# LepistaBioinformatics/blutils

Measured on AMD Instinct MI355X. Metric: Mqueries/sec consensus (synthetic outfmt-6 hit table), higher is better.
Workload: dtype i32/u32

## Files before the change

### blutils_amd/csrc/consensus_kernel.hip

```cpp

#if defined(__HIP_DEVICE_COMPILE__) && !defined(__gfx950__)
#error "consensus_kernel.hip is written for gfx950"
#endif

#include <hip/hip_runtime.h>

#include <climits>
#include <cstdint>
#include <type_traits>

#include "blu_internal.h"

namespace blu {

#define WAVE 64

constexpr int BLOCK_A = 768;
constexpr int BLU_WAVES_PER_SIMD = 3;
constexpr int BLOCK_N = 1024;
constexpr int BLU_N_WAVES_PER_SIMD = 4;
constexpr int BLOCK_F = 704;
constexpr int LIST_CAP = 208;
constexpr int LIST_CAP_F64 = 232;
constexpr uint32_t SHORT_SEG = 128u;
constexpr uint32_t MAX_TASK_SEG = 512u;
constexpr uint32_t BLU_LONG_COST = 96u;
constexpr uint32_t BLU_DENSE_Q = 3u;
constexpr int BLU_STEP_SETS = 2;
constexpr uint32_t FLAT_ROWS = 8u;
constexpr uint32_t FLAT_SEG = 64u * FLAT_ROWS;
constexpr uint32_t FLAT_STEPS = 8u;
constexpr uint32_t FLAT_DEPTH = 4u;
constexpr uint32_t RING_ROWS = 2048u;
constexpr uint32_t RING_PAD = 32u;
constexpr uint32_t RING_CHUNKS = RING_ROWS / 256u;
constexpr uint32_t RING_MASK = RING_ROWS - 1u;
constexpr int STREAM_AUX = 0;
#define RING_DMA_MOD " sc1 nt"
constexpr int GATHER_AUX = 2;
constexpr int RECORD_AUX = 18;
constexpr int BLOCK_B = 256;
constexpr int BLU_B_WAVES_PER_SIMD = 7;

__device__ __forceinline__ int lane_id() { return (int)__builtin_amdgcn_mbcnt_hi(~0u, __builtin_amdgcn_mbcnt_lo(~0u, 0u)); }

template <int CTRL>
__device__ __forceinline__ int dpp(int v) { return __builtin_amdgcn_update_dpp(0, v, CTRL, 0xF, 0xF, true); }

#define ROW_REDUCE(x, OP)            \
    x = OP(x, dpp<0xB1>(x));         \
    x = OP(x, dpp<0x4E>(x));         \
    x = OP(x, dpp<0x124>(x));        \
    x = OP(x, dpp<0x128>(x));

__device__ __forceinline__ int imax(int a, int b) { return a > b ? a : b; }
__device__ __forceinline__ int imin(int a, int b) { return a < b ? a : b; }
__device__ __forceinline__ uint32_t umin(uint32_t a, uint32_t b) { return a < b ? a : b; }
__device__ __forceinline__ int rl(int v, int lane) { return __builtin_amdgcn_readlane(v, lane); }

__device__ __forceinline__ int wave_max_i32(int x) {
    ROW_REDUCE(x, imax)
    return imax(imax(rl(x, 0), rl(x, 16)), imax(rl(x, 32), rl(x, 48)));
}
__device__ __forceinline__ int wave_min_i32(int x) {
    ROW_REDUCE(x, imin)
    return imin(imin(rl(x, 0), rl(x, 16)), imin(rl(x, 32), rl(x, 48)));
}
__device__ __forceinline__ int iadd(int a, int b) { return a + b; }
__device__ __forceinline__ int wave_sum_u32(uint32_t v) {
    int x = (int)v;
    ROW_REDUCE(x, iadd)
    return rl(x, 0) + rl(x, 16) + rl(x, 32) + rl(x, 48);
}
__device__ __forceinline__ uint32_t wave_max_u32(uint32_t v) { return (uint32_t)wave_max_i32((int)(v ^ 0x80000000u)) ^ 0x80000000u; }
__device__ __forceinline__ uint32_t wave_min_u32(uint32_t v) { return (uint32_t)wave_min_i32((int)(v ^ 0x80000000u)) ^ 0x80000000u; }

__device__ __forceinline__ uint32_t wave_incl_scan_u32(uint32_t v) {
    uint32_t incl = v;
    incl += (uint32_t)dpp<0x111>((int)incl);
    incl += (uint32_t)dpp<0x112>((int)incl);
    incl += (uint32_t)dpp<0x114>((int)incl);
    incl += (uint32_t)dpp<0x118>((int)incl);
    const uint32_t t0 = (uint32_t)rl((int)incl, 15), t1 = (uint32_t)rl((int)incl, 31), t2 = (uint32_t)rl((int)incl, 47);
    const uint32_t r16 = (uint32_t)lane_id() >> 4;
    return incl + (r16 == 0 ? 0u : (r16 == 1 ? t0 : (r16 == 2 ? t0 + t1 : t0 + t1 + t2)));
}
#define WL_QUEUES 64u
#define WL_BASE 64u
#define WL_STRIDE 32u
__device__ __forceinline__ uint32_t wl_capacity(uint64_t n_queries) {
    const uint64_t n_tasks = (n_queries + WAVE - 1) / WAVE;
    return (uint32_t)((n_tasks + WL_QUEUES - 1) / WL_QUEUES) * WAVE;
}
__device__ __forceinline__ void wl_push(uint32_t* const wl_q, uint32_t* const wl_cnt, const uint32_t q) {
    __hip_atomic_store(wl_q + atomicAdd(wl_cnt, 1u), q, __ATOMIC_RELAXED, __HIP_MEMORY_SCOPE_AGENT);
}
__device__ __forceinline__ uint32_t wl_entry(const uint32_t* __restrict__ worklist, const uint32_t cap, const uint32_t incl, const uint32_t wi) {
    const uint32_t sub = (uint32_t)__builtin_popcountll(__ballot(incl <= wi));
    const uint32_t before = sub ? (uint32_t)rl((int)incl, (int)sub - 1) : 0u;
    return __hip_atomic_load(worklist + (uint64_t)sub * cap + (wi - before), __ATOMIC_RELAXED, __HIP_MEMORY_SCOPE_AGENT);
}

template <int CTRL>
__device__ __forceinline__ double dpp_f64(double v) {
    return __hiloint2double(dpp<CTRL>(__double2hiint(v)), dpp<CTRL>(__double2loint(v)));
}
__device__ __forceinline__ double rl_f64(double v, int lane) {
    return __hiloint2double(rl(__double2hiint(v), lane), rl(__double2loint(v), lane));
}
__device__ __forceinline__ double dmax(double a, double b) { return b > a ? b : a; }
__device__ __forceinline__ double dmin(double a, double b) { return b < a ? b : a; }
__device__ __forceinline__ double wave_max_f64(double x) {
    x = dmax(x, dpp_f64<0xB1>(x)); x = dmax(x, dpp_f64<0x4E>(x));
    x = dmax(x, dpp_f64<0x124>(x)); x = dmax(x, dpp_f64<0x128>(x));
    return dmax(dmax(rl_f64(x, 0), rl_f64(x, 16)), dmax(rl_f64(x, 32), rl_f64(x, 48)));
}
__device__ __forceinline__ double wave_min_f64(double x) {
    x = dmin(x, dpp_f64<0xB1>(x)); x = dmin(x, dpp_f64<0x4E>(x));
    x = dmin(x, dpp_f64<0x124>(x)); x = dmin(x, dpp_f64<0x128>(x));
    return dmin(dmin(rl_f64(x, 0), rl_f64(x, 16)), dmin(rl_f64(x, 32), rl_f64(x, 48)));
}
__device__ __forceinline__ int first_lane(uint64_t m) { return __builtin_ctzll(m); }
__device__ __forceinline__ int last_lane(uint64_t m) { return 63 - __builtin_clzll(m); }
__device__ __forceinline__ uint64_t rl_u64(uint64_t v, int lane) {
    return (uint64_t)(uint32_t)rl((int)(uint32_t)v, lane) | ((uint64_t)(uint32_t)rl((int)(uint32_t)(v >> 32), lane) << 32);
}
__device__ __forceinline__ uint64_t uniform64(uint64_t v) {
    return (uint64_t)(uint32_t)__builtin_amdgcn_readfirstlane((uint32_t)v) |
           ((uint64_t)(uint32_t)__builtin_amdgcn_readfirstlane((uint32_t)(v >> 32)) << 32);
}

__device__ __forceinline__ void store_result(blu_result* out, uint64_t q, uint32_t status, uint32_t flags,
                                             uint32_t bean_index, uint32_t mar_level, uint32_t reached_rank,
                                             uint32_t mar_code, uint32_t identifier, uint32_t ref_row,
                                             uint64_t level_mask, double ident) {
    uint4 a;
    a.x = (status & 0xFF) | ((flags & 0xFF) << 8) | ((bean_index & 0xFF) << 16) | ((mar_level & 0xFF) << 24);
    a.y = (reached_rank & 0xFFFF) | ((mar_code & 0xFFFF) << 16);
    a.z = identifier;
    a.w = ref_row;
    uint4 b;
    b.x = (uint32_t)level_mask;
    b.y = (uint32_t)(level_mask >> 32);
    b.z = (uint32_t)__double2loint(ident);
    b.w = (uint32_t)__double2hiint(ident);
    uint4* p = reinterpret_cast<uint4*>(out + q);
    p[0] = a;
    p[1] = b;
}
__device__ __forceinline__ void pack_result(uint4& a, uint4& b, uint32_t status, uint32_t flags, uint32_t bean_index,
                                            uint32_t mar_level, uint32_t reached_rank, uint32_t mar_code, uint32_t identifier,
                                            uint32_t ref_row, uint64_t level_mask, double ident) {
    a.x = (status & 0xFF) | ((flags & 0xFF) << 8) | ((bean_index & 0xFF) << 16) | ((mar_level & 0xFF) << 24);
    a.y = (reached_rank & 0xFFFF) | ((mar_code & 0xFFFF) << 16);
    a.z = identifier;
    a.w = ref_row;
    b.x = (uint32_t)level_mask;
    b.y = (uint32_t)(level_mask >> 32);
    b.z = (uint32_t)__double2loint(ident);
    b.w = (uint32_t)__double2hiint(ident);
}
__device__ __forceinline__ void pack_status(uint4& a, uint4& b, uint32_t status, uint32_t ref_row) {
    pack_result(a, b, status, 0, BLU_NONE_U8, BLU_NONE_U8, BLU_NONE_U16, BLU_NONE_U16, 0xFFFFFFFFu, ref_row, 0ull, 0.0);
}
__device__ __forceinline__ void store_status(blu_result* out, uint64_t q, uint32_t status, uint32_t ref_row) {
    store_result(out, q, status, 0, BLU_NONE_U8, BLU_NONE_U8, BLU_NONE_U16, BLU_NONE_U16, 0xFFFFFFFFu, ref_row, 0ull, 0.0);
}

__device__ __forceinline__ double milli_to_f64(uint32_t k) { return (double)k / 1000.0; }
__device__ __forceinline__ double milli17_to_f64(uint32_t k) {
    const double x = (double)k, y = 0.001;
    const double q = x * y;
    const double r = __builtin_fma(-q, 1000.0, x);
    return __builtin_fma(r, y, q);
}

__device__ __forceinline__ uint32_t packed_rank(uint32_t p) { return (p >> BLU_PACK_CUT_BITS) & BLU_PACK_CODE_MASK; }
__device__ __forceinline__ uint32_t packed_mar(uint32_t p) {
    const uint32_t m = p >> (BLU_PACK_CUT_BITS + BLU_PACK_CODE_BITS);
    return m == BLU_PACK_NEVER ? BLU_MAR_NEVER_EQUAL : m;
// ... 608 lines not shown
                    const uint32_t oq = g - L.qs[q];
                    left = g < total ? (int)sg.y - (int)(UR * oq) : 0;
                    if (left > 0) { voff = (sg.x + UR * oq) * 4u; um = q | (oq << 6) | (umin((uint32_t)left, UR) << 12); }
                }
                lo4 = __builtin_amdgcn_raw_buffer_load_b128(rs_bs, voff, 0, STREAM_AUX);
                hi4 = __builtin_amdgcn_raw_buffer_load_b128(rs_bs, left > 4 ? voff + 16u : 0xFFFFFFF0u, 0, STREAM_AUX);
            };
            u32x4 ba[DEPTH], bb[DEPTH];
            uint32_t um[MAXS];
            int lmx[MAXS];
#pragma unroll
            for (uint32_t st = 0; st < MAXS; ++st) { um[st] = 0u; lmx[st] = INT_MIN; }
#pragma unroll
            for (uint32_t st = 0; st < DEPTH; ++st) issue(st, ba[st], bb[st], um[st]);
#pragma unroll
            for (uint32_t st = 0; st < MAXS; ++st) {
                if (st >= ns) break;
                const u32x4 va = ba[st % DEPTH], vb = bb[st % DEPTH];
                const uint32_t left = (um[st] >> 12) & 15u;
                const uint32_t v[8] = {va.x, va.y, va.z, va.w, vb.x, vb.y, vb.z, vb.w};
                int bsv[UR], mx = INT_MIN;
#pragma unroll
                for (uint32_t r = 0; r < UR; ++r) { bsv[r] = left > r ? (int)v[r] : INT_MIN; mx = imax(mx, bsv[r]); }
                uint32_t lmask = 0;
#pragma unroll
                for (uint32_t r = 0; r < UR; ++r) lmask |= (uint32_t)(left > r && bsv[r] == mx) << r;
                um[st] |= lmask << 16;
                lmx[st] = mx;
                if (left) atomicMax(&L.qm[um[st] & 63u], mx);
                if (st + DEPTH < MAXS) issue(st + DEPTH, ba[st % DEPTH], bb[st % DEPTH], um[st + DEPTH]);
            }
            __builtin_amdgcn_fence(__ATOMIC_RELEASE, "workgroup");
            __builtin_amdgcn_wave_barrier();
            __builtin_amdgcn_fence(__ATOMIC_ACQUIRE, "workgroup");
            uint32_t running = fill, q_cut = q_lim;
#pragma unroll
            for (uint32_t st = 0; st < MAXS; ++st) {
                if (st >= ns) break;
                const uint32_t q = um[st] & 63u, oq = (um[st] >> 6) & 63u;
                const bool have = ((um[st] >> 12) & 15u) != 0u;
                const int M = L.qm[q];
                const uint32_t tmask = (have && lmx[st] == M) ? (um[st] >> 16) & 0xFFu : 0u;
                const uint32_t c = (uint32_t)__builtin_popcount(tmask);
                uint32_t in2 = c;
                in2 += (uint32_t)dpp<0x111>((int)in2);
                in2 += (uint32_t)dpp<0x112>((int)in2);
                in2 += (uint32_t)dpp<0x114>((int)in2);
                in2 += (uint32_t)dpp<0x118>((int)in2);
                const uint32_t k0 = (uint32_t)rl((int)in2, 15), k1 = (uint32_t)rl((int)in2, 31), k2 = (uint32_t)rl((int)in2, 47), k3 = (uint32_t)rl((int)in2, 63);
                in2 += r16 == 0 ? 0u : (r16 == 1 ? k0 : (r16 == 2 ? k0 + k1 : k0 + k1 + k2));
                const uint32_t idx0 = running + in2 - c;
                if (have && oq == 0u) L.meta[q] = META_SLOW | idx0;
                if (c) atomicAdd(&L.qk[q], c);
                const bool over = have && idx0 + c > CAP;
                const uint64_t over_m = __ballot(over);
                const bool room = !over && c != 0u && (over_m == 0ull || (uint32_t)lane < (uint32_t)__builtin_ctzll(over_m));
                if (room) L.rec[idx0] = make_uint4(__builtin_bitreverse32(tmask), L.seg[q].x + UR * oq, UR * oq, 0u);
                if (over_m) { q_cut = (uint32_t)rl((int)q, __builtin_ctzll(over_m)); break; }
                running += k0 + k1 + k2 + k3;
            }
            __builtin_amdgcn_fence(__ATOMIC_RELEASE, "workgroup");
            __builtin_amdgcn_wave_barrier();
            __builtin_amdgcn_fence(__ATOMIC_ACQUIRE, "workgroup");
            const uint32_t m = L.meta[lane];
            if (rows != 0u && (uint32_t)lane < q_cut) L.meta[lane] = (m & 0xFFFFu) | (L.qk[lane] << 16);
            fill = q_cut < q_lim ? (L.meta[q_cut] & 0xFFFFu) : running;
            if (q_cut < WAVE) stop_q = q_cut;
            }
        };
        auto ring_mark_landed = [&](const uint32_t upto) {
            const uint32_t m0 = (ring_landed + RING_CHUNKS - 1u) & ~(RING_CHUNKS - 1u);
            if (m0 < upto) {
                if ((uint32_t)lane < RING_PAD) L.ring[RING_ROWS + lane] = L.ring[lane];
                __builtin_amdgcn_fence(__ATOMIC_RELEASE, "workgroup");
                __builtin_amdgcn_wave_barrier();
                __builtin_amdgcn_fence(__ATOMIC_ACQUIRE, "workgroup");
            }
            ring_landed = upto;
        };
        auto ring_refill = [&]() {
            if (ring_head < ring_tail) { ring_head = ring_tail; if (ring_landed < ring_tail) ring_landed = ring_tail; }
            const uint32_t lim = ring_end < ring_tail + RING_CHUNKS ? ring_end : ring_tail + RING_CHUNKS;
            if (ring_head < lim) { ring_dma_run(rs_ring, ring_c0, ring_head, lim); ring_head = lim; }
        };
        auto phase1_scan = [&](const auto rpl_c, const auto full_c, const uint32_t LPQ) {
            constexpr uint32_t RPL = decltype(rpl_c)::value;
            constexpr bool FULL = decltype(full_c)::value;
            static_assert(RPL <= RING_PAD && RPL <= 32u, "rows per lane");
            const uint32_t QPS = WAVE / LPQ;
            const uint32_t grp = (uint32_t)lane / LPQ, sub = ((uint32_t)lane & (LPQ - 1u)) * RPL, row16 = (uint32_t)lane >> 4;
            {
                const uint32_t cs = (uint32_t)((vbase + (uint32_t)rl((int)seg_x, (int)first_q)) >> 8);
                if (cs < ring_tail) { wait_vmcnt(0u); ring_head = ring_landed = ring_tail = cs; }
            }
            for (uint32_t qb = first_q / QPS * QPS; qb < nq; qb += QPS) {
                const uint32_t r_lo = (uint32_t)rl((int)seg_x, (int)(qb < first_q ? first_q : qb));
                const uint32_t qn = qb + QPS;
                const uint32_t r_hi = qn < nq ? (uint32_t)rl((int)seg_x, (int)qn) : task_nrows;
                ring_tail = (uint32_t)((vbase + r_lo) >> 8);
                ring_refill();
                if (r_hi > r_lo) {
                    const uint32_t need = (uint32_t)((vbase + r_hi - 1u) >> 8);
                    if (need >= ring_landed) { wait_vmcnt(ring_head - 1u - need); ring_mark_landed(need + 1u); }
                }
                const uint32_t qi = qb + grp;
                const uint2 sg = L.seg[qi];
                const int left0 = (sg.y > short_seg ? 0 : (int)sg.y) - (int)sub;
                const uint32_t over = (FULL && left0 > 0 && left0 < (int)RPL) ? RPL - (uint32_t)left0 : 0u;
                const uint32_t sub_e = sub - over;
                const int left = FULL ? (left0 > 0 ? (int)RPL : 0) : left0;
                const uint32_t row0 = sg.x + sub_e;
                const uint32_t a = ((uint32_t)vbase + L.vx[qi] + sub_e) & RING_MASK;
                int b[RPL];
#pragma unroll
                for (uint32_t i = 0; i < RPL; ++i) b[i] = (int)L.ring[a + i];
                asm volatile("s_waitcnt lgkmcnt(0)" ::: "memory");
#pragma unroll
                for (uint32_t i = 0; i < RPL; ++i) asm volatile("" : "+v"(b[i]));
                if (r_hi > r_lo) { ring_tail = (uint32_t)((vbase + r_hi) >> 8); ring_refill(); }
                int M = INT_MIN;
                if constexpr (FULL) {
#pragma unroll
                    for (uint32_t i = 0; i < RPL; ++i) M = imax(M, b[i]);
                    M = left > 0 ? M : INT_MIN;
                } else {
#pragma unroll
                    for (uint32_t i = 0; i < RPL; ++i) { b[i] = (int)i < left ? b[i] : INT_MIN; M = imax(M, b[i]); }
                }
                if (LPQ >= 2) M = imax(M, dpp<0xB1>(M));
                if (LPQ >= 4) M = imax(M, dpp<0x4E>(M));
                if (LPQ >= 8) M = imax(M, dpp<0x141>(M));
                if (LPQ >= 16) M = imax(M, dpp<0x140>(M));
                uint32_t mask = tie_mask<RPL>(b, M);
                mask = left > 0 ? mask : 0u;
                if constexpr (FULL) mask &= 0xFFFFFFFFu >> (32u - RPL + over);
                const uint32_t c = (uint32_t)__builtin_popcount(mask);
                uint32_t incl = c;
                incl += (uint32_t)dpp<0x111>((int)incl);
                incl += (uint32_t)dpp<0x112>((int)incl);
                incl += (uint32_t)dpp<0x114>((int)incl);
                incl += (uint32_t)dpp<0x118>((int)incl);
                const uint32_t k0 = (uint32_t)rl((int)incl, 15), k1 = (uint32_t)rl((int)incl, 31);
                const uint32_t k2 = (uint32_t)rl((int)incl, 47), k3 = (uint32_t)rl((int)incl, 63);
                const bool fits = fill + k0 + k1 + k2 + k3 <= CAP;
                const uint32_t p1 = fill + k0, p2 = p1 + k1, p3 = p2 + k2;
                const uint32_t rbase = row16 == 0 ? fill : (row16 == 1 ? p1 : (row16 == 2 ? p2 : p3));
                uint32_t gk = c;
                if (LPQ >= 2) gk += (uint32_t)dpp<0xB1>((int)gk);
                if (LPQ >= 4) gk += (uint32_t)dpp<0x4E>((int)gk);
                if (LPQ >= 8) gk += (uint32_t)dpp<0x141>((int)gk);
                if (LPQ >= 16) gk += (uint32_t)dpp<0x140>((int)gk);
                if (PID32 && !fits) {
                    __builtin_amdgcn_s_setprio(2);
                    uint64_t BK = 0;
                    uint32_t bacc = 0, bpos = 0, brow = 0, kmin = 0xFFFFFFFFu, pmax = 0, dlo = 0xFFFFFFFFu, dhi = 0, err = 0xFFFFFFFFu;
                    auto reset = [&]() { BK = 0; bacc = 0; bpos = 0; brow = 0; kmin = 0xFFFFFFFFu; pmax = 0; dlo = 0xFFFFFFFFu; dhi = 0; err = 0xFFFFFFFFu; };
                    auto better = [&](const uint64_t K, const uint32_t acc, const uint32_t pos, const uint64_t K2, const uint32_t acc2, const uint32_t pos2) {
                        const bool gt = (K > K2) | ((K == K2) & (acc > acc2)), eq = (K == K2) & (acc == acc2);
                        return STRAT == BLU_RELAXED ? (gt | (eq & (pos > pos2))) : ((!gt & !eq) | (eq & (pos < pos2)));
                    };
                    auto take_record = [&](const u32x4 rec, const uint32_t gp, const bool on) {
                        const uint32_t len = umin(rec.x >> BLU_ROW_BITS, t.max_depth), pos = rec.x & ROW_MASK;
                        const bool unmatched = pos >= t.n_tax, bad = !unmatched && (rec.x >> BLU_ROW_BITS) == 0;
                        const uint32_t e = (gp << 8) | (bad ? (uint32_t)BLU_ST_ERR_BAD_LINEAGE : (uint32_t)BLU_ST_ERR_UNMATCHED_TAXID);
                        err = (on && (unmatched | bad)) ? umin(err, e) : err;
                        const uint32_t pm = rec.y & ((1u << KEY_PID_BITS) - 1u);
                        const uint32_t k1 = (len << KEY_PID_BITS) | pm;
                        const uint64_t K = ((uint64_t)k1 << 32) | (rec.z ^ 0x80000000u);
                        const bool take = on & ((kmin == 0xFFFFFFFFu) | better(K, rec.w, gp, BK, bacc, bpos));
                        BK = take ? K : BK; bacc = take ? rec.w : bacc; bpos = take ? gp : bpos; brow = take ? pos : brow;
                        kmin = on ? umin(kmin, k1) : kmin;
                        const uint32_t pmo = pm | ((!PACKED && rec.y >= (1u << KEY_PID_BITS)) ? 0x80000000u : 0u);
                        pmax = (on && pmo > pmax) ? pmo : pmax;
                        dlo = on ? umin(dlo, pos) : dlo;
                        dhi = (on && pos > dhi) ? pos : dhi;
                    };
                    auto load_record = [&](const uint32_t row, const bool on) {
                        u32x4 r;
                        if (PACKED) r = __builtin_amdgcn_raw_buffer_load_b128(rs_tax, on ? row * 16u : 0xFFFFFFC0u, 0, GATHER_AUX);
                        else {
                            const uint32_t o4 = on ? row * 4u : 0xFFFFFFF0u;
                            r.x = __builtin_amdgcn_raw_buffer_load_b32(rs_tax, o4, 0, GATHER_AUX);
                            r.y = __builtin_amdgcn_raw_buffer_load_b32(rs_pid, o4, 0, GATHER_AUX);
                            r.z = __builtin_amdgcn_raw_buffer_load_b32(rs_aln, o4, 0, GATHER_AUX);
                            r.w = __builtin_amdgcn_raw_buffer_load_b32(rs_acc, o4, 0, GATHER_AUX);
                        }
                        return r;
                    };
                    auto merge = [&](auto ctrl) {
                        constexpr int C = decltype(ctrl)::value;
                        const uint64_t K2 = ((uint64_t)(uint32_t)dpp<C>((int)(uint32_t)(BK >> 32)) << 32) | (uint32_t)dpp<C>((int)(uint32_t)BK);
                        const uint32_t acc2 = (uint32_t)dpp<C>((int)bacc), pos2 = (uint32_t)dpp<C>((int)bpos), row2 = (uint32_t)dpp<C>((int)brow);
                        const uint32_t kmin2 = (uint32_t)dpp<C>((int)kmin);
                        const bool take = (kmin2 != 0xFFFFFFFFu) & ((kmin == 0xFFFFFFFFu) | better(K2, acc2, pos2, BK, bacc, bpos));
                        BK = take ? K2 : BK; bacc = take ? acc2 : bacc; bpos = take ? pos2 : bpos; brow = take ? row2 : brow;
                        kmin = umin(kmin, kmin2);
                        const uint32_t pm2 = (uint32_t)dpp<C>((int)pmax); pmax = pm2 > pmax ? pm2 : pmax;
                        dlo = umin(dlo, (uint32_t)dpp<C>((int)dlo));
                        const uint32_t hi2 = (uint32_t)dpp<C>((int)dhi); dhi = hi2 > dhi ? hi2 : dhi;
                        err = umin(err, (uint32_t)dpp<C>((int)err));
                    };
                    auto deliver = [&](const int src, const bool mine) {
                        const uint32_t f_khi = (uint32_t)__builtin_amdgcn_ds_bpermute(src, (int)(uint32_t)(BK >> 32));
                        const uint32_t f_pos = (uint32_t)__builtin_amdgcn_ds_bpermute(src, (int)bpos), f_row = (uint32_t)__builtin_amdgcn_ds_bpermute(src, (int)brow);
                        const uint32_t f_kmin = (uint32_t)__builtin_amdgcn_ds_bpermute(src, (int)kmin), f_pmax = (uint32_t)__builtin_amdgcn_ds_bpermute(src, (int)pmax);
                        const uint32_t f_lo = (uint32_t)__builtin_amdgcn_ds_bpermute(src, (int)dlo), f_hi = (uint32_t)__builtin_amdgcn_ds_bpermute(src, (int)dhi);
                        const uint32_t f_err = (uint32_t)__builtin_amdgcn_ds_bpermute(src, (int)err);
                        const bool got = mine && f_kmin != 0xFFFFFFFFu;
                        const bool g_ovf = got && (f_pmax & 0x80000000u) != 0u, g_err = got && !g_ovf && f_err != 0xFFFFFFFFu, g_ok = got && !g_ovf && !g_err;
                        dn_flag = g_ovf ? 3u : (g_err ? 2u : (g_ok ? 1u : dn_flag));
                        dn_err = g_err ? (f_err & 0xFFu) : dn_err;
                        dn_pos = g_err ? (f_err >> 8) : dn_pos;
                        if constexpr (PID32) { r_pid = g_ok ? (f_khi & ((1u << KEY_PID_BITS) - 1u)) : r_pid; max_pid = g_ok ? f_pmax : max_pid; }
                        r_len = g_ok ? (f_khi >> KEY_PID_BITS) : r_len; r_row = g_ok ? f_row : r_row; r_pos = g_ok ? f_pos : r_pos;
                        minlen = g_ok ? (f_kmin >> KEY_PID_BITS) : minlen; g_lo = g_ok ? f_lo : g_lo; g_hi = g_ok ? f_hi : g_hi;
                    };
                    const uint32_t tq = (uint32_t)lane;
                    const bool mine = tq >= qb && tq < qn && tq < nq;
                    const uint32_t own0 = (mine ? tq - qb : 0u) * LPQ;
                    if (LPQ <= 4u && BLU_DENSE_Q * (k0 + k1 + k2 + k3) >= r_hi - r_lo) {
                        const uint32_t c4 = (uint32_t)lane & 3u;
#pragma nounroll
                        for (uint32_t g = 0; g < 4u; ++g) {
                            const int own = (int)((16u * g + ((uint32_t)lane >> 2)) * 4u);
                            const uint32_t o_row0 = (uint32_t)__builtin_amdgcn_ds_bpermute(own, (int)row0);
                            const uint32_t o_mask = (uint32_t)__builtin_amdgcn_ds_bpermute(own, (int)mask);
                            const uint32_t o_sub = (uint32_t)__builtin_amdgcn_ds_bpermute(own, (int)sub_e);
                            if (__ballot(o_mask != 0u) == 0ull) continue;
                            reset();
                            constexpr uint32_t NF = PACKED ? 4u : 2u;
#pragma unroll
                            for (uint32_t b0 = 0; b0 < RPL; b0 += 4u * NF) {
                                if (__ballot(((o_mask >> (RPL - 4u * NF - b0)) & ((1u << (4u * NF)) - 1u)) != 0u) == 0ull) continue;
                                u32x4 rq[NF];
#pragma unroll
                                for (uint32_t j = 0; j < NF; ++j) {
                                    const uint32_t i = b0 + 4u * j + c4;
                                    rq[j] = load_record(o_row0 + i, ((o_mask >> (RPL - 1u - i)) & 1u) != 0u);
                                }
#pragma unroll
                                for (uint32_t j = 0; j < NF; ++j) {
                                    const uint32_t i = b0 + 4u * j + c4;
                                    take_record(rq[j], o_sub + i, ((o_mask >> (RPL - 1u - i)) & 1u) != 0u);
                                }
                            }
                            merge(std::integral_constant<int, 0xB1>());
                            merge(std::integral_constant<int, 0x4E>());
                            if (LPQ >= 2) merge(std::integral_constant<int, 0x141>());
                            if (LPQ >= 4) merge(std::integral_constant<int, 0x140>());
                            deliver((int)(((own0 & 15u) * 4u) * 4u), mine && (own0 >> 4) == g);
                        }
                    } else {
                        uint32_t m = mask;
                        while (__ballot(m != 0u)) {
                            u32x4 rq[4];
                            uint32_t gp[4];
#pragma unroll
                            for (int j = 0; j < 4; ++j) {
                                const bool on = m != 0u;
                                const uint32_t hb = on ? 31u - (uint32_t)__builtin_clz(m) : 0u, i = RPL - 1u - hb;
                                m = on ? (m & ~(1u << hb)) : 0u;
                                gp[j] = on ? sub_e + i : 0xFFFFFFFFu;
                                rq[j] = load_record(row0 + i, on);
                            }
#pragma unroll
                            for (int j = 0; j < 4; ++j) take_record(rq[j], gp[j], gp[j] != 0xFFFFFFFFu);
                        }
                        if (LPQ >= 2) merge(std::integral_constant<int, 0xB1>());
                        if (LPQ >= 4) merge(std::integral_constant<int, 0x4E>());
                        if (LPQ >= 8) merge(std::integral_constant<int, 0x141>());
                        if (LPQ >= 16) merge(std::integral_constant<int, 0x140>());
                        deliver((int)(own0 * 4u), mine);
                    }
                    {
                        const uint32_t f_gk = (uint32_t)__builtin_amdgcn_ds_bpermute((int)(own0 * 4u), (int)gk);
                        dn_k = (mine && dn_flag == 1u) ? f_gk : dn_k;
                    }
                    if (sub == 0 && gk != 0u) L.meta[qi] = META_DENSE;
                    __builtin_amdgcn_s_setprio(0);
                    continue;
                }
                uint32_t idx = rbase + incl - c;
                if (!fits) {
                    const uint32_t lane_o = (uint32_t)__builtin_ctzll(__ballot(idx + c > CAP));
                    const uint32_t qo = qb + lane_o / LPQ;
                    const bool taken = qi < qo;
                    if (sub == 0) L.meta[qi] = taken ? (idx | (gk << 16)) : META_SLOW;
                    if (taken && c) { L.rec[idx].x = mask << (32u - RPL); L.rec[idx].y = DESC_WORD1(RPL, row0, sub_e); }
                    fill = (uint32_t)rl((int)idx, (int)((qo - qb) * LPQ));
                    stop_q = qo;
                    wait_vmcnt(0u);
                    ring_head = ring_landed = ring_tail = (uint32_t)((vbase + (uint32_t)rl((int)seg_x, (int)qo)) >> 8);
                    break;
                }
                if (sub == 0) L.meta[qi] = idx | (gk << 16);
                fill = p3 + k3;
                static_assert((RPL == 16u || RPL == 32u) && SHORT_SEG <= 128u, "descriptor word of a lane");
                if (c) { L.rec[idx].x = mask << (32u - RPL); L.rec[idx].y = DESC_WORD1(RPL, row0, sub_e); }
            }
        };
        auto gather_list = [&](auto&& between) {
            constexpr int NG = (CAP + WAVE - 1) / WAVE;
            u32x4 g[NG];
            uint32_t ghi[NG], gpos[NG], ghint[NG];
            uint32_t carry = 0;
#pragma unroll
            for (int u = 0; u < NG; ++u) {
                g[u] = u32x4{0u, 0u, 0u, 0u}; ghi[u] = 0u; gpos[u] = 0u; ghint[u] = 0u;
                if ((uint32_t)u * WAVE >= fill_ring) continue;
                const uint32_t idx = (uint32_t)u * WAVE + (uint32_t)lane;
                const bool valid = idx < fill_ring;
                const uint32_t d0 = L.rec[idx < CAP ? idx : 0u].x;
                int s = (valid && d0 != 0u) ? (int)idx : 0;
                s = imax(s, dpp<0x111>(s));
                s = imax(s, dpp<0x112>(s));
                s = imax(s, dpp<0x114>(s));
                s = imax(s, dpp<0x118>(s));
                s = imax(s, __builtin_amdgcn_update_dpp(0, s, 0x142, 0xA, 0xF, false));
                s = imax(s, __builtin_amdgcn_update_dpp(0, s, 0x143, 0xC, 0xF, false));
                s = imax(s, (int)carry);
                carry = (uint32_t)rl(s, 63);
                const uint4 dd = L.rec[s];
                const uint32_t d0w = dd.x, d = dd.y;
                uint32_t r = idx - (uint32_t)s, x = scan_rpl == 32u ? d0w : d0w >> 16, i = 0;
                if (scan_rpl == 32u) {
                    const uint32_t h = x >> 16, ch = (uint32_t)__builtin_popcount(h);
                    const bool low = r >= ch;
                    r -= low ? ch : 0u; x = low ? (x & 0xFFFFu) : h; i += low ? 16u : 0u;
                }
                {
                    const uint32_t h = x >> 8, ch = (uint32_t)__builtin_popcount(h);
                    const bool low = r >= ch;
                    r -= low ? ch : 0u; x = low ? (x & 0xFFu) : h; i += low ? 8u : 0u;
                }
                {
                    const uint32_t h = x >> 4, ch = (uint32_t)__builtin_popcount(h);
                    const bool low = r >= ch;
                    r -= low ? ch : 0u; x = low ? (x & 0xFu) : h; i += low ? 4u : 0u;
                }
                {
                    const uint32_t h = x >> 2, ch = (uint32_t)__builtin_popcount(h);
                    const bool low = r >= ch;
                    r -= low ? ch : 0u; x = low ? (x & 0x3u) : h; i += low ? 2u : 0u;
                }
                i += (r >= (x >> 1)) ? 1u : 0u;
                const uint32_t row = (RING ? (d >> DESC_SUB_BITS) : d) + i;
                gpos[u] = (RING ? (d & ((1u << DESC_SUB_BITS) - 1u)) : dd.z) + i;
                if (PACKED) g[u] = __builtin_amdgcn_raw_buffer_load_b128(rs_tax, valid ? row * 16u : 0xFFFFFFC0u, 0, GATHER_AUX);
                else if (WIDE) {
                    g[u] = __builtin_amdgcn_raw_buffer_load_b128(rs_tax, valid ? row * 24u : 0xFFFFFFC0u, 0, GATHER_AUX);
                    const u32x2 p = __builtin_amdgcn_raw_buffer_load_b64(rs_tax, valid ? row * 24u + 16u : 0xFFFFFFE0u, 0, GATHER_AUX);
                    ghint[u] = g[u].y;
                    g[u].y = p.x; ghi[u] = p.y;
                } else {
                    const uint32_t o4 = valid ? row * 4u : 0xFFFFFFF0u;
                    g[u].x = __builtin_amdgcn_raw_buffer_load_b32(rs_tax, o4, 0, GATHER_AUX);
                    if (PID32) g[u].y = __builtin_amdgcn_raw_buffer_load_b32(rs_pid, o4, 0, GATHER_AUX);
                    else {
                        const u32x2 p = __builtin_amdgcn_raw_buffer_load_b64(rs_pid, valid ? row * 8u : 0xFFFFFFE0u, 0, GATHER_AUX);
                        g[u].y = p.x; ghi[u] = p.y;
                    }
                    g[u].z = __builtin_amdgcn_raw_buffer_load_b32(rs_aln, o4, 0, GATHER_AUX);
                    g[u].w = __builtin_amdgcn_raw_buffer_load_b32(rs_acc, o4, 0, GATHER_AUX);
                }
            }
            between();
            bool ovf = false;
            uint32_t gk[NG];
#pragma unroll
            for (int u = 0; u < NG; ++u) {
                const bool valid = (uint32_t)u * WAVE + (uint32_t)lane < fill_ring;
                if constexpr (PID32) { gk[u] = g[u].y & PM_MASK; ovf |= !PACKED && valid && g[u].y >= (1u << KEY_PID_BITS); }
                else {
                    const double p = __hiloint2double((int)ghi[u], (int)g[u].y);
                    const bool in_range = p >= 0.0 && p < 131.0705;
                    const uint32_t k = in_range ? (uint32_t)(p * 1000.0 + 0.5) : 0u;
                    const double back = milli17_to_f64(k);
                    gk[u] = k;
                    ovf |= valid && !(in_range && __double2hiint(back) == (int)ghi[u] && __double2loint(back) == (int)g[u].y && k < BLU_KTHR_NEVER);
                }
            }
            keyed = __ballot(ovf) == 0ull && fill == fill_ring;
            bool any_bad = false;
#pragma unroll
            for (int u = 0; u < NG; ++u) {
                const uint32_t idx = (uint32_t)u * WAVE + (uint32_t)lane;
                if (idx < fill_ring) {
                    if (keyed) {
                        const uint32_t len = umin(g[u].x >> BLU_ROW_BITS, t.max_depth);
                        any_bad |= len == 0u || (g[u].x & ROW_MASK) >= t.n_tax;
                        const uint32_t hint = (PID32 ? g[u].y : ghint[u]) >> KEY_PID_BITS;
                        L.rec[idx] = make_uint4((g[u].x & ROW_MASK) | ((hint >> 8) << BLU_ROW_BITS),
                                                (len << KEYED_LEN_SHIFT) | (gk[u] << KEYED_PID_SHIFT) | (hint & 0xFFu), g[u].z ^ 0x80000000u, g[u].w);
                    } else L.rec[idx] = make_uint4(g[u].x, g[u].y, g[u].z, g[u].w);
                    L.pq[idx] = (uint16_t)gpos[u];
                    if (!PID32) L.p1[idx] = ghi[u];
                }
            }
            keyed_bad = __ballot(any_bad) != 0ull;
        };
        bool pend = (uint32_t)lane < nq;
        uint32_t pend_before = WAVE + 1;
        if (RING && contiguous) {
            ring_c0 = (uint32_t)(vbase >> 8);
            rs_ring = ring_desc(ring_c0);
            ring_end = task_nrows ? (uint32_t)((vbase + task_nrows - 1u) >> 8) + 1u : ring_c0;
            if (pref_q0 != q0_32) ring_head = ring_landed = ring_c0;
            ring_tail = ring_c0;
        }
        for (;;) {
        fill = 0;
        stop_q = WAVE;
        bool ring_round = false;
        bool list_round = false;
        keyed = false;
        {
            const uint32_t rows = L.seg[lane].y;
            const uint64_t live = __ballot(rows != 0u);
            first_q = live ? (uint32_t)__builtin_ctzll(live) : 0u;
// ... 868 lines not shown
```

Before: 11370.

## Software-pipeline dense-step record gathers and balance sparse gathers across lane pairs

The dense path of the overflow step now runs one continuous loop over all owner groups, using a three-deep ring of record requests so loads for the next blocks are in flight while the current block is reduced. The running best result is packed into fewer registers (position and row share one word, max pid and min length share another), which cuts the cross-lane DPP and bpermute traffic during merge and deliver. The sparse path pairs adjacent lanes so each gathers half of the pair's hits from both ends, and it issues a configurable number of loads per round. In exchange the code is more complex, register pressure from the ring buffer rises, and correctness depends on the new bit-packing assumptions, which are guarded by static asserts.

New measurement: 11260. About the same (-0.9%).

```diff
diff --git a/blutils_amd/csrc/consensus_kernel.hip b/blutils_amd/csrc/consensus_kernel.hip
--- a/blutils_amd/csrc/consensus_kernel.hip
+++ b/blutils_amd/csrc/consensus_kernel.hip
@@ -26,6 +26,10 @@
 constexpr uint32_t MAX_TASK_SEG = 512u;
 constexpr uint32_t BLU_LONG_COST = 96u;
 constexpr uint32_t BLU_DENSE_Q = 3u;
+#ifndef BLU_SPARSE_REQ_X
+#define BLU_SPARSE_REQ_X 6u
+#endif
+constexpr uint32_t BLU_SPARSE_REQ = BLU_SPARSE_REQ_X;
 constexpr int BLU_STEP_SETS = 2;
 constexpr uint32_t FLAT_ROWS = 8u;
 constexpr uint32_t FLAT_SEG = 64u * FLAT_ROWS;
@@ -940,9 +944,15 @@
                 if (LPQ >= 16) gk += (uint32_t)dpp<0x140>((int)gk);
                 if (PID32 && !fits) {
                     __builtin_amdgcn_s_setprio(2);
+                    constexpr uint32_t PL_LEN_SHIFT = KEY_PID_BITS + 1u, PL_PID_MASK = (1u << PL_LEN_SHIFT) - 1u;
+                    static_assert(BLU_ROW_BITS + 7u <= 32u && SHORT_SEG <= 128u && PL_LEN_SHIFT + 7u <= 32u, "packed words of a dense step's running result");
                     uint64_t BK = 0;
-                    uint32_t bacc = 0, bpos = 0, brow = 0, kmin = 0xFFFFFFFFu, pmax = 0, dlo = 0xFFFFFFFFu, dhi = 0, err = 0xFFFFFFFFu;
-                    auto reset = [&]() { BK = 0; bacc = 0; bpos = 0; brow = 0; kmin = 0xFFFFFFFFu; pmax = 0; dlo = 0xFFFFFFFFu; dhi = 0; err = 0xFFFFFFFFu; };
+                    uint32_t bacc = 0, bw = 0, pl = 0, dlo = 0xFFFFFFFFu, dhi = 0, err = 0xFFFFFFFFu;
+                    auto reset = [&]() { BK = 0; bacc = 0; bw = 0; pl = 0; dlo = 0xFFFFFFFFu; dhi = 0; err = 0xFFFFFFFFu; };
+                    auto pl_max = [&](const uint32_t a, const uint32_t b) {
+                        const uint32_t pa = a & PL_PID_MASK, pb = b & PL_PID_MASK, la = a >> PL_LEN_SHIFT, lb = b >> PL_LEN_SHIFT;
+                        return (pa > pb ? pa : pb) | ((la > lb ? la : lb) << PL_LEN_SHIFT);
+                    };
                     auto better = [&](const uint64_t K, const uint32_t acc, const uint32_t pos, const uint64_t K2, const uint32_t acc2, const uint32_t pos2) {
                         const bool gt = (K > K2) | ((K == K2) & (acc > acc2)), eq = (K == K2) & (acc == acc2);
                         return STRAT == BLU_RELAXED ? (gt | (eq & (pos > pos2))) : ((!gt & !eq) | (eq & (pos < pos2)));
@@ -955,11 +965,11 @@
                         const uint32_t pm = rec.y & ((1u << KEY_PID_BITS) - 1u);
                         const uint32_t k1 = (len << KEY_PID_BITS) | pm;
                         const uint64_t K = ((uint64_t)k1 << 32) | (rec.z ^ 0x80000000u);
-                        const bool take = on & ((kmin == 0xFFFFFFFFu) | better(K, rec.w, gp, BK, bacc, bpos));
-                        BK = take ? K : BK; bacc = take ? rec.w : bacc; bpos = take ? gp : bpos; brow = take ? pos : brow;
-                        kmin = on ? umin(kmin, k1) : kmin;
-                        const uint32_t pmo = pm | ((!PACKED && rec.y >= (1u << KEY_PID_BITS)) ? 0x80000000u : 0u);
-                        pmax = (on && pmo > pmax) ? pmo : pmax;
+                        const uint32_t w = pos | (gp << BLU_ROW_BITS);
+                        const bool take = on & ((dlo == 0xFFFFFFFFu) | better(K, rec.w, w, BK, bacc, bw));
+                        BK = take ? K : BK; bacc = take ? rec.w : bacc; bw = take ? w : bw;
+                        const uint32_t pmo = pm | ((!PACKED && rec.y >= (1u << KEY_PID_BITS)) ? (1u << KEY_PID_BITS) : 0u);
+                        pl = on ? pl_max(pl, pmo | ((127u - len) << PL_LEN_SHIFT)) : pl;
                         dlo = on ? umin(dlo, pos) : dlo;
                         dhi = (on && pos > dhi) ? pos : dhi;
                     };
@@ -978,81 +988,123 @@
                     auto merge = [&](auto ctrl) {
                         constexpr int C = decltype(ctrl)::value;
                         const uint64_t K2 = ((uint64_t)(uint32_t)dpp<C>((int)(uint32_t)(BK >> 32)) << 32) | (uint32_t)dpp<C>((int)(uint32_t)BK);
-                        const uint32_t acc2 = (uint32_t)dpp<C>((int)bacc), pos2 = (uint32_t)dpp<C>((int)bpos), row2 = (uint32_t)dpp<C>((int)brow);
-                        const uint32_t kmin2 = (uint32_t)dpp<C>((int)kmin);
-                        const bool take = (kmin2 != 0xFFFFFFFFu) & ((kmin == 0xFFFFFFFFu) | better(K2, acc2, pos2, BK, bacc, bpos));
-                        BK = take ? K2 : BK; bacc = take ? acc2 : bacc; bpos = take ? pos2 : bpos; brow = take ? row2 : brow;
-                        kmin = umin(kmin, kmin2);
-                        const uint32_t pm2 = (uint32_t)dpp<C>((int)pmax); pmax = pm2 > pmax ? pm2 : pmax;
-                        dlo = umin(dlo, (uint32_t)dpp<C>((int)dlo));
+                        const uint32_t acc2 = (uint32_t)dpp<C>((int)bacc), w2 = (uint32_t)dpp<C>((int)bw);
+                        const uint32_t lo2 = (uint32_t)dpp<C>((int)dlo);
+                        const bool take = (lo2 != 0xFFFFFFFFu) & ((dlo == 0xFFFFFFFFu) | better(K2, acc2, w2, BK, bacc, bw));
+                        BK = take ? K2 : BK; bacc = take ? acc2 : bacc; bw = take ? w2 : bw;
+                        pl = pl_max(pl, (uint32_t)dpp<C>((int)pl));
+                        dlo = umin(dlo, lo2);
                         const uint32_t hi2 = (uint32_t)dpp<C>((int)dhi); dhi = hi2 > dhi ? hi2 : dhi;
                         err = umin(err, (uint32_t)dpp<C>((int)err));
                     };
                     auto deliver = [&](const int src, const bool mine) {
                         const uint32_t f_khi = (uint32_t)__builtin_amdgcn_ds_bpermute(src, (int)(uint32_t)(BK >> 32));
-                        const uint32_t f_pos = (uint32_t)__builtin_amdgcn_ds_bpermute(src, (int)bpos), f_row = (uint32_t)__builtin_amdgcn_ds_bpermute(src, (int)brow);
-                        const uint32_t f_kmin = (uint32_t)__builtin_amdgcn_ds_bpermute(src, (int)kmin), f_pmax = (uint32_t)__builtin_amdgcn_ds_bpermute(src, (int)pmax);
+                        const uint32_t f_w = (uint32_t)__builtin_amdgcn_ds_bpermute(src, (int)bw), f_pl = (uint32_t)__builtin_amdgcn_ds_bpermute(src, (int)pl);
+                        const uint32_t f_pos = f_w >> BLU_ROW_BITS, f_row = f_w & ROW_MASK, f_pmax = f_pl & ((1u << KEY_PID_BITS) - 1u);
                         const uint32_t f_lo = (uint32_t)__builtin_amdgcn_ds_bpermute(src, (int)dlo), f_hi = (uint32_t)__builtin_amdgcn_ds_bpermute(src, (int)dhi);
                         const uint32_t f_err = (uint32_t)__builtin_amdgcn_ds_bpermute(src, (int)err);
-                        const bool got = mine && f_kmin != 0xFFFFFFFFu;
-                        const bool g_ovf = got && (f_pmax & 0x80000000u) != 0u, g_err = got && !g_ovf && f_err != 0xFFFFFFFFu, g_ok = got && !g_ovf && !g_err;
+                        const bool got = mine && f_lo != 0xFFFFFFFFu;
+                        const bool g_ovf = got && (f_pl & (1u << KEY_PID_BITS)) != 0u, g_err = got && !g_ovf && f_err != 0xFFFFFFFFu, g_ok = got && !g_ovf && !g_err;
                         dn_flag = g_ovf ? 3u : (g_err ? 2u : (g_ok ? 1u : dn_flag));
                         dn_err = g_err ? (f_err & 0xFFu) : dn_err;
                         dn_pos = g_err ? (f_err >> 8) : dn_pos;
                         if constexpr (PID32) { r_pid = g_ok ? (f_khi & ((1u << KEY_PID_BITS) - 1u)) : r_pid; max_pid = g_ok ? f_pmax : max_pid; }
                         r_len = g_ok ? (f_khi >> KEY_PID_BITS) : r_len; r_row = g_ok ? f_row : r_row; r_pos = g_ok ? f_pos : r_pos;
-                        minlen = g_ok ? (f_kmin >> KEY_PID_BITS) : minlen; g_lo = g_ok ? f_lo : g_lo; g_hi = g_ok ? f_hi : g_hi;
+                        minlen = g_ok ? 127u - (f_pl >> PL_LEN_SHIFT) : minlen; g_lo = g_ok ? f_lo : g_lo; g_hi = g_ok ? f_hi : g_hi;
                     };
                     const uint32_t tq = (uint32_t)lane;
                     const bool mine = tq >= qb && tq < qn && tq < nq;
                     const uint32_t own0 = (mine ? tq - qb : 0u) * LPQ;
+                    const uint32_t lane_at = DESC_WORD1(RPL, row0, sub_e);
                     if (LPQ <= 4u && BLU_DENSE_Q * (k0 + k1 + k2 + k3) >= r_hi - r_lo) {
                         const uint32_t c4 = (uint32_t)lane & 3u;
+                        constexpr uint32_t NH = 2u;
+                        constexpr uint32_t BPO = RPL / (4u * NH);
+                        constexpr uint32_t NBLK = 4u * BPO;
+                        static_assert(BPO >= 2u && BPO % 2u == 0u, "a group of owners ends at an odd block; three blocks span at most two groups");
+                        struct Owner { uint32_t mask, at; };
+                        auto owner_of = [&](const uint32_t g) {
+                            const int own = (int)((16u * (g & 3u) + ((uint32_t)lane >> 2)) * 4u);
+                            Owner o;
+                            o.mask = (uint32_t)__builtin_amdgcn_ds_bpermute(own, (int)mask);
+                            o.at = (uint32_t)__builtin_amdgcn_ds_bpermute(own, (int)lane_at);
+                            o.mask = g < 4u ? o.mask : 0u;
+                            return o;
+                        };
+                        auto request = [&](u32x4 (&rq)[NH], const Owner& o, const uint32_t b0) {
+#pragma unroll
+                            for (uint32_t j = 0; j < NH; ++j) {
+                                const uint32_t i = b0 + 4u * j + c4;
+                                rq[j] = load_record((o.at >> DESC_SUB_BITS) + i, ((o.mask >> (RPL - 1u - i)) & 1u) != 0u);
+                            }
+                        };
+                        auto reduce = [&](const u32x4 (&rq)[NH], const Owner& o, const uint32_t b0) {
+                            if (__ballot(((o.mask >> (RPL - 4u * NH - b0)) & ((1u << (4u * NH)) - 1u)) != 0u) == 0ull) return;
+#pragma unroll
+                            for (uint32_t j = 0; j < NH; ++j) {
+                                const uint32_t i = b0 + 4u * j + c4;
+                                take_record(rq[j], (o.at & ((1u << DESC_SUB_BITS) - 1u)) + i, ((o.mask >> (RPL - 1u - i)) & 1u) != 0u);
+                            }
+                        };
+                        u32x4 rq[3][NH];
+                        Owner oc = owner_of(0u), on = oc;
+                        request(rq[0], oc, 0u);
+                        request(rq[1], oc, 4u * NH);
+                        reset();
 #pragma nounroll
-                        for (uint32_t g = 0; g < 4u; ++g) {
-                            const int own = (int)((16u * g + ((uint32_t)lane >> 2)) * 4u);
-                            const uint32_t o_row0 = (uint32_t)__builtin_amdgcn_ds_bpermute(own, (int)row0);
-                            const uint32_t o_mask = (uint32_t)__builtin_amdgcn_ds_bpermute(own, (int)mask);
-                            const uint32_t o_sub = (uint32_t)__builtin_amdgcn_ds_bpermute(own, (int)sub_e);
-                            if (__ballot(o_mask != 0u) == 0ull) continue;
-                            reset();
-                            constexpr uint32_t NF = PACKED ? 4u : 2u;
-#pragma unroll
-                            for (uint32_t b0 = 0; b0 < RPL; b0 += 4u * NF) {
-                                if (__ballot(((o_mask >> (RPL - 4u * NF - b0)) & ((1u << (4u * NF)) - 1u)) != 0u) == 0ull) continue;
-                                u32x4 rq[NF];
-#pragma unroll
-                                for (uint32_t j = 0; j < NF; ++j) {
-                                    const uint32_t i = b0 + 4u * j + c4;
-                                    rq[j] = load_record(o_row0 + i, ((o_mask >> (RPL - 1u - i)) & 1u) != 0u);
-                                }
-#pragma unroll
-                                for (uint32_t j = 0; j < NF; ++j) {
-                                    const uint32_t i = b0 + 4u * j + c4;
-                                    take_record(rq[j], o_sub + i, ((o_mask >> (RPL - 1u - i)) & 1u) != 0u);
+                        for (uint32_t h0 = 0; h0 < NBLK; h0 += 6u) {
+#pragma unroll
+                            for (uint32_t u = 0; u < 6u; ++u) {
+                                const uint32_t hb = h0 + u, nb = hb + 2u;
+                                if (nb % BPO == 0u) on = owner_of(nb / BPO);
+                                request(rq[(u + 2u) % 3u], on, (nb % BPO) * 4u * NH);
+                                reduce(rq[u % 3u], oc, (hb % BPO) * 4u * NH);
+                                if ((u & 1u) != 0u && hb % BPO == BPO - 1u) {
+                                    if (__ballot(oc.mask != 0u) != 0ull) {
+                                        merge(std::integral_constant<int, 0xB1>());
+                                        merge(std::integral_constant<int, 0x4E>());
+                                        if (LPQ >= 2) merge(std::integral_constant<int, 0x141>());
+                                        if (LPQ >= 4) merge(std::integral_constant<int, 0x140>());
+                                        deliver((int)(((own0 & 15u) * 4u) * 4u), mine && (own0 >> 4) == hb / BPO);
+                                    }
+                                    reset();
+                                    oc = on;
                                 }
                             }
-                            merge(std::integral_constant<int, 0xB1>());
-                            merge(std::integral_constant<int, 0x4E>());
-                            if (LPQ >= 2) merge(std::integral_constant<int, 0x141>());
-                            if (LPQ >= 4) merge(std::integral_constant<int, 0x140>());
-                            deliver((int)(((own0 & 15u) * 4u) * 4u), mine && (own0 >> 4) == g);
                         }
                     } else {
-                        uint32_t m = mask;
-                        while (__ballot(m != 0u)) {
-                            u32x4 rq[4];
-                            uint32_t gp[4];
-#pragma unroll
-                            for (int j = 0; j < 4; ++j) {
-                                const bool on = m != 0u;
-                                const uint32_t hb = on ? 31u - (uint32_t)__builtin_clz(m) : 0u, i = RPL - 1u - hb;
-                                m = on ? (m & ~(1u << hb)) : 0u;
-                                gp[j] = on ? sub_e + i : 0xFFFFFFFFu;
-                                rq[j] = load_record(row0 + i, on);
+                        const bool back = LPQ >= 2u && ((uint32_t)lane & 1u) != 0u;
+                        uint32_t m_own = mask, m_oth = 0u, at_oth = 0u, todo = c;
+                        if (LPQ >= 2u) {
+                            m_oth = (uint32_t)dpp<0xB1>((int)mask);
+                            at_oth = (uint32_t)dpp<0xB1>((int)lane_at);
+                            const uint32_t pair = c + (uint32_t)__builtin_popcount(m_oth);
+                            todo = back ? pair / 2u : pair - pair / 2u;
+                        }
+                        while (__ballot(todo != 0u)) {
+                            constexpr uint32_t NR = BLU_SPARSE_REQ;
+                            u32x4 rq[NR];
+                            uint32_t gpw[(NR + 3u) / 4u];
+#pragma unroll
+                            for (uint32_t j = 0; j < (NR + 3u) / 4u; ++j) gpw[j] = 0u;
+#pragma unroll
+                            for (uint32_t j = 0; j < NR; ++j) {
+                                const bool on = todo != 0u, own = m_own != 0u;
+                                const uint32_t mm = (own ? m_own : m_oth) | (on ? 0u : 1u);
+                                const uint32_t hb = back ? (uint32_t)__builtin_ctz(mm) : 31u - (uint32_t)__builtin_clz(mm);
+                                const uint32_t i = RPL - 1u - hb;
+                                const uint32_t at = own ? lane_at : at_oth;
+                                m_own = (on && own) ? (m_own & ~(1u << hb)) : m_own;
+                                m_oth = (on && !own) ? (m_oth & ~(1u << hb)) : m_oth;
+                                todo -= on ? 1u : 0u;
+                                gpw[j / 4u] |= (on ? (at & ((1u << DESC_SUB_BITS) - 1u)) + i : 0xFFu) << (8u * (j % 4u));
+                                rq[j] = load_record((at >> DESC_SUB_BITS) + i, on);
                             }
 #pragma unroll
-                            for (int j = 0; j < 4; ++j) take_record(rq[j], gp[j], gp[j] != 0xFFFFFFFFu);
+                            for (uint32_t j = 0; j < NR; ++j) {
+                                const uint32_t gp = (gpw[j / 4u] >> (8u * (j % 4u))) & 0xFFu;
+                                take_record(rq[j], gp, gp != 0xFFu);
+                            }
                         }
                         if (LPQ >= 2) merge(std::integral_constant<int, 0xB1>());
                         if (LPQ >= 4) merge(std::integral_constant<int, 0x4E>());
```
